# bittremieux/ANN-SoLo

Measured on AMD Instinct MI355X. Metric: query spectra/sec + recall@k vs brute-force, open-mod search on MassIVE-KB, higher is better.
Workload: dtype f32; 1 GPU; configs[2]: MassIVE-KB-scale synthetic library (2100000 spectra, one charge-2 partition), ivfpq m=32 nlist=4096 nprobe=128 k=1024, open +-500 Da, shifted dot, fragment tol 0.02 Da; library_size=2100000, batch_per_gpu=32768, reference_default_batch_size=16384, global_batch=32768, index=ivfpq, nlist=4096, nprobe=128, k=1024, parallelism=single

## Files before the change

ann_solo_amd/csrc/pq_scan_v3.hip:

```cpp
#include "common.hpp"
#include "hist_topk.hpp"
#include "ivf_kernels.hpp"
#include "pq_tile.hpp"

namespace asl {

constexpr int V3_CHUNK = 256;
constexpr int V3_DEPTH = 1;
constexpr int V3_NT = 0;
constexpr int V3_AHEAD = 8;
constexpr uint32_t V3_MM_DEAD = 0xfffffff0u;
constexpr int V3_PAD_SALU = 0;
constexpr int V3_PAD_VALU = 0;
#define V3_PAD4(op) op " %0, 0\n\t" op " %1, 1\n\t" op " %2, 2\n\t" op " %3, 3\n\t"
#define V3_PAD16(op) V3_PAD4(op) V3_PAD4(op) V3_PAD4(op) V3_PAD4(op)
template <int NS_, int NV_>
__device__ __forceinline__ void v3_pad() {
  static_assert(NS_ % 16 == 0 && NV_ % 16 == 0, "the padding comes in blocks of 16 instructions");
#pragma unroll
  for (int n = 0; n < NS_ / 16; ++n) {
    uint32_t a, b, c, d;
    asm volatile(V3_PAD16("s_mov_b32") : "=s"(a), "=s"(b), "=s"(c), "=s"(d));
  }
#pragma unroll
  for (int n = 0; n < NV_ / 16; ++n) {
    uint32_t a, b, c, d;
    asm volatile(V3_PAD16("v_mov_b32") : "=v"(a), "=v"(b), "=v"(c), "=v"(d));
  }
}
#undef V3_PAD16
#undef V3_PAD4
constexpr int V3_PAD_LDSRT = 0;
template <int N_>
__device__ __forceinline__ void v3_pad_ldsrt(const int *word) {
  if constexpr (N_ > 0) {
    typedef __attribute__((address_space(3))) int lds_int;
    uint32_t a = (uint32_t)(uintptr_t)(const lds_int *)word;
#pragma unroll
    for (int n = 0; n < N_; ++n) {
      const int r = __builtin_amdgcn_readfirstlane(
          __hip_atomic_load((const lds_int *)(uintptr_t)a, __ATOMIC_RELAXED, __HIP_MEMORY_SCOPE_WORKGROUP));
      asm volatile("" : "+v"(a) : "s"(r));
    }
  }
}
constexpr int V3_WAVES_PER_SIMD = 6;

template <int NT_>
__device__ __forceinline__ uint4 load_codes16(const uint8_t *p) {
  if (NT_) {
    const uint32_t *w = reinterpret_cast<const uint32_t *>(p);
    typedef uint32_t u32x4 __attribute__((ext_vector_type(4)));
    const u32x4 v = __builtin_nontemporal_load(reinterpret_cast<const u32x4 *>(w));
    return make_uint4(v.x, v.y, v.z, v.w);
  }
  return *reinterpret_cast<const uint4 *>(p);
}

struct TileEnt8 {
  uint32_t tile_nv;
  float coarse;
};

struct TileEnt12 {
  uint32_t tile_nv;
  float coarse;
  uint32_t first;
};
constexpr int V3_CHUNK_RANGED = 168;
static_assert(V3_CHUNK_RANGED * sizeof(TileEnt12) <= V3_CHUNK * sizeof(TileEnt8), "the ranged table fits the 2 KB");

template <int CAP, int T, int NW, int DEPTH, bool WIDE, bool RANGED = false, bool SEL = false, bool MM = false>
__global__ __launch_bounds__(64 * NW, (NW == 8 ? (CAP <= 2048 ? V3_WAVES_PER_SIMD : 4) : (CAP <= 2048 ? 3 : 1))) void pq_scan_v3_kernel(
    const float *__restrict__ xq, int d, const float *__restrict__ codebooks, int dsub,
    const float *__restrict__ coarse_D, const int32_t *__restrict__ coarse_I, int nprobe,
    const int32_t *__restrict__ list_offsets, const int32_t *__restrict__ tile_offsets,
    const uint8_t *__restrict__ codes_tiled, const int32_t *__restrict__ ids_tiled, int k,
    float *__restrict__ D, int64_t *__restrict__ I64, int32_t *__restrict__ I32, int set_mode,
    const uint2 *__restrict__ ent, const int32_t *__restrict__ ent_cnt, const int *__restrict__ gate,
    const ScanPostFilter pf, const ScanRanges rg, const unsigned long long *__restrict__ sel, const uint32_t mm_plane) {
  static_assert(!SEL || CAP <= 2048, "the selector is built into the 2048-key instantiations only");
  static_assert(!MM || (!RANGED && !SEL), "the sub-quantiser-major copy exists of the default layout only");
  if (gate && (int)blockIdx.x >= *gate) return;
  static_assert(DEPTH >= 1 && DEPTH <= 3, "rounds of prefetch");
  static_assert(T == 1, "one tile per wave at a time (two lost on registers: profiles/HISTORY.md)");
  constexpr int NT = 64 * NW, ROUND_VECS = NW * 64;
  using TopK = HistTopK<CAP, ROUND_VECS, NT>;
  using Ent = typename std::conditional<RANGED, TileEnt12, TileEnt8>::type;
  extern __shared__ __attribute__((aligned(16))) char smem[];
  float *s_lut = reinterpret_cast<float *>(smem + TopK::lds_bytes());
  Ent *table = reinterpret_cast<Ent *>(s_lut + PQT_KSUB * PQT_M);
  float *s_q = reinterpret_cast<float *>(smem);

  const int tid = threadIdx.x, lane = tid & 63, wave = tid >> 6, q = blockIdx.x;
  constexpr int PP = WIDE ? 2 : 1;
  int my_len[PP], my_tile0[PP], my_nt[PP], my_pre[PP];
  float my_coarse[PP];
#pragma unroll
  for (int pp = 0; pp < PP; ++pp) {
    my_len[pp] = 0, my_tile0[pp] = 0, my_nt[pp] = 0, my_coarse[pp] = 0.0f;
    const int p = tid + pp * NT;
    if (p < nprobe) {
      const int l = coarse_I[(size_t)q * nprobe + p];
      if (l >= 0) {
        if constexpr (RANGED) {
          const int2 r = rg.range[(size_t)q * nprobe + p];
          my_len[pp] = r.y > r.x ? r.y - (r.x & ~63) : 0;
          my_tile0[pp] = (int)((uint32_t)(tile_offsets[l] + (r.x >> 6)) | ((uint32_t)(r.x & 63) << 26));
        } else {
          my_len[pp] = list_offsets[l + 1] - list_offsets[l];
          my_tile0[pp] = tile_offsets[l];
        }
        my_nt[pp] = (my_len[pp] + 63) >> 6;
        my_coarse[pp] = coarse_D[(size_t)q * nprobe + p];
      }
    }
  }
  build_lut_cbt<NT>(xq + (size_t)q * d, d, codebooks, dsub, s_q, s_lut, reinterpret_cast<uint8_t *>(table),
                    tid, ent ? ent + (size_t)q * 64 : nullptr,
                    ent ? (xq ? ent_cnt[q] : max(ent_cnt[q], 0)) : -1);

  uint32_t live_u = 0;
  if constexpr (MM) {
    const uint8_t *s_nz = reinterpret_cast<const uint8_t *>(table);
    const int K = reinterpret_cast<const int *>(s_nz)[0];
    uint32_t mine = 0;
    for (int i = tid & 63; i < K; i += 64) mine |= 1u << (s_nz[8 + i] & 31);
#pragma unroll
    for (int o = 32; o > 0; o >>= 1) mine |= (uint32_t)__shfl_xor((int)mine, o);
    live_u = (uint32_t)__builtin_amdgcn_readfirstlane((int)mine);
    __syncthreads();
  }

  int total = 0;
  int *scan_part = reinterpret_cast<int *>(table);
#pragma unroll
  for (int pp = 0; pp < PP; ++pp) {
    int part_total;
    my_pre[pp] = total + block_excl_scan<NW>(my_nt[pp], scan_part, tid, part_total);
    total += part_total;
    __syncthreads();
  }
  total = __builtin_amdgcn_readfirstlane(total);

  TopK top;
  top.init(smem, k, ids_tiled, tid);
  top.out_keys = set_mode == 2 && I64 != nullptr;

  const char *lut_bytes = reinterpret_cast<const char *>(s_lut);
  const int wave_u = __builtin_amdgcn_readfirstlane(wave);
  const int rho = lane >> 4, j = lane & 15;
  const int ma = (rho & 1) ? j + 16 : j, mb = ma ^ 16;
  const uint32_t offA = (uint32_t)ma * 4u, offB = (uint32_t)mb * 4u;
  const bool liveA = (live_u >> ma) & 1u, liveB = (live_u >> mb) & 1u;
  const uint32_t chunkA = MM ? (liveA ? (uint32_t)ma * mm_plane + (uint32_t)(rho * 16) : V3_MM_DEAD) : (uint32_t)(rho * 512 + ma * 16);
  const uint32_t chunkB = liveB ? (uint32_t)mb * mm_plane + (uint32_t)(rho * 16) : V3_MM_DEAD;

  int *s_flag = top.ctl + TopK::C_USER;
  int *s_done = top.ctl + TopK::C_USER + 1;
  if (tid == 0) {
    *s_flag = 0;
    *s_done = 0;
  }
  auto flag_up = [&]() -> int { return __hip_atomic_load(s_flag, __ATOMIC_RELAXED, __HIP_MEMORY_SCOPE_WORKGROUP); };
  auto flag_set = [&](int v) { __hip_atomic_store(s_flag, v, __ATOMIC_RELAXED, __HIP_MEMORY_SCOPE_WORKGROUP); };
  float thr_u = -INFINITY;
  uint32_t thr_hi_u = 0;
  int flag_u = 0;

  constexpr int CHUNK = RANGED ? V3_CHUNK_RANGED : V3_CHUNK;
  for (int c0 = 0; c0 < total; c0 += CHUNK) {
#pragma unroll
    for (int pp = 0; pp < PP; ++pp) {
      asm volatile("" : "+v"(my_pre[pp]), "+v"(my_tile0[pp]), "+v"(my_len[pp]));
      const int lo = max(my_pre[pp], c0), hi = min(my_pre[pp] + ((my_len[pp] + 63) >> 6), c0 + CHUNK);
      for (int t = lo; t < hi; ++t) {
        const int local = t - my_pre[pp];
        Ent e;
        const uint32_t tile0 = RANGED ? (uint32_t)my_tile0[pp] & 0x3ffffffu : (uint32_t)my_tile0[pp];
        e.tile_nv = (tile0 + (uint32_t)local) | ((uint32_t)(min(64, my_len[pp] - local * 64) - 1) << 26);
        e.coarse = my_coarse[pp];
        if constexpr (RANGED) e.first = local == 0 ? (uint32_t)my_tile0[pp] >> 26 : 0u;
        table[t - c0] = e;
      }
    }
    __syncthreads();
    const int nent = min(CHUNK, total - c0);
    constexpr int NS = DEPTH + 1;
    uint4 A[NS], B[NS];
    if constexpr (MM) {
#pragma unroll
      for (int s = 0; s < NS; ++s) A[s] = B[s] = make_uint4(0u, 0u, 0u, 0u);
    }
    struct Tile {
      uint32_t tile_nv;
      float coarse;
      uint32_t first;
      unsigned long long sel;
    } e[NS];
    auto fetch = [&](uint32_t taddr, uint4 &a, uint4 &b, Tile &en, uint32_t num_records = 0) {
      typedef uint32_t u32x2 __attribute__((ext_vector_type(2)));
      const u32x2 t = *(const __attribute__((address_space(3))) u32x2 *)(uintptr_t)taddr;
      en.tile_nv = __builtin_amdgcn_readfirstlane(t.x);
      en.coarse = __builtin_bit_cast(float, __builtin_amdgcn_readfirstlane((int)t.y));
      if constexpr (RANGED)
        en.first = __builtin_amdgcn_readfirstlane(*(const __attribute__((address_space(3))) uint32_t *)(uintptr_t)(taddr + 8u));
      if constexpr (SEL) en.sel = sel[en.tile_nv & 0x3ffffffu];
      if constexpr (MM) {
        const uint32_t toff = (en.tile_nv & 0x3ffffffu) * 64u;
        const uint8_t *base = codes_tiled + (size_t)toff;
        const __amdgpu_buffer_rsrc_t rs =
            __builtin_amdgcn_make_buffer_rsrc(const_cast<uint8_t *>(base), 0, (int)num_records, 0x00020000);
        typedef uint32_t u32x4 __attribute__((ext_vector_type(4)));
        const u32x4 va = __builtin_amdgcn_raw_buffer_load_b128(rs, (int)chunkA, 0, V3_NT ? 2 : 0);
        const u32x4 vb = __builtin_amdgcn_raw_buffer_load_b128(rs, (int)chunkB, 0, V3_NT ? 2 : 0);
        a = make_uint4(va.x, va.y, va.z, va.w);
        b = make_uint4(vb.x, vb.y, vb.z, vb.w);
      } else {
        const uint8_t *base = codes_tiled + (size_t)(en.tile_nv & 0x3ffffffu) * 2048;
        uint32_t offa = chunkA;
        asm volatile("" : "+v"(offa));
        const uint32_t offb = offa ^ 256u;
        a = load_codes16<V3_NT>(base + offa);
        b = load_codes16<V3_NT>(base + offb);
      }
    };
    constexpr uint32_t ENT_STRIDE = NW * sizeof(Ent);
    const uint32_t mm_size = (uint32_t)PQT_M * mm_plane;
    float p_score = 0.0f;
    uint32_t p_tile_nv = 0, p_first = 0;
    unsigned long long p_sel = 0;
    bool pending = false;
    auto in_mask = [&]() -> unsigned long long {
      unsigned long long in = ~0ull >> (~(p_tile_nv >> 26) & 63u);
      if constexpr (RANGED) in &= ~0ull << (p_first & 63u);
      if constexpr (SEL) in &= p_sel;
      return in;
    };
    auto passers = [&]() -> unsigned long long { return __ballot(p_score >= thr_u) & in_mask(); };
    auto append = [&](unsigned long long m, bool hot = false) {
      if (!hot && thr_hi_u != 0) {
        float sc = p_score;
        asm volatile("; exact flushes" : "+v"(sc));
        m = __ballot(f2ord(sc) >= thr_hi_u) & in_mask();
      }
      pending = false;
      if (hot || m) {
        const int c = __builtin_amdgcn_readfirstlane(__popcll(m));
        const int base = top.reserve_add(c);
        pending = base + c > CAP;
        if (!pending) top.free_write(__builtin_amdgcn_inverse_ballot_w64(m), m, p_score, (p_tile_nv << 6) + (uint32_t)lane, base, false);
      }
    };
    const uint32_t table_lds = (uint32_t)(uintptr_t)(const __attribute__((address_space(3))) char *)reinterpret_cast<const char *>(table);
    int i = wave_u;
    if (i < nent) {
      uint32_t t0 = table_lds + (uint32_t)i * (uint32_t)sizeof(Ent);
      asm volatile("" : "+v"(t0));
#pragma unroll
      for (int s = 0; s < DEPTH; ++s)
        if (i + s * NW < nent) fetch(t0 + s * ENT_STRIDE, A[s], B[s], e[s], mm_size);
    }
    uint32_t taddr = 0;
    auto step = [&](int s) {
      const int f = (s + DEPTH) % NS;
      const int fl = flag_up();
      const bool real = i + DEPTH * NW < nent;
      if constexpr (MM) {
        taddr += real ? ENT_STRIDE : 0u;
        fetch(taddr, A[f], B[f], e[f], real ? mm_size : 0u);
      } else if (real) {
        taddr += ENT_STRIDE;
        fetch(taddr, A[f], B[f], e[f]);
      }
      flag_u = __builtin_amdgcn_readfirstlane(fl);
      p_score = e[s].coarse + tile_adc<V3_AHEAD>(lut_bytes, A[s], B[s], offA, offB);
      p_tile_nv = e[s].tile_nv;
      if constexpr (RANGED) p_first = e[s].first;
      if constexpr (SEL) p_sel = e[s].sel;
      i += NW;
    };
    auto hot = [&]() -> int {
      for (;;) {
#pragma unroll
        for (int s = 0; s < NS; ++s) {
          if (i >= nent) return -1;
          step(s);
          v3_pad<V3_PAD_SALU, V3_PAD_VALU>();
          v3_pad_ldsrt<V3_PAD_LDSRT>(s_done);
          const unsigned long long m = passers();
          if (__builtin_expect(((uint32_t)m | (uint32_t)(m >> 32) | (uint32_t)flag_u | thr_hi_u) != 0u, 0)) {
            if (((uint32_t)flag_u | thr_hi_u) != 0u) return s;
            append(m, true);
            if (pending) return s + NS;
          }
        }
      }
    };
    bool finished = false;
    for (;;) {
      taddr = table_lds + (uint32_t)(DEPTH == 1 ? min(i, CHUNK - 1) : min(i + (DEPTH - 1) * NW, nent - 1)) * (uint32_t)sizeof(Ent);
      asm volatile("" : "+v"(taddr));
      int ev = hot();
      asm volatile("" : "+s"(ev));
      bool meet = false;
#pragma unroll
      for (int s = 0; s < NS; ++s) {
        if (ev < 0 || s < ev % NS || meet) continue;
        if (s > ev % NS) {
          if (i >= nent) continue;
          step(s);
        }
        if (!(ev >= NS && s == ev % NS)) append(passers());
        if (pending || flag_u) {
          meet = true;
          if (s + 1 < NS) {
#pragma unroll
            for (int u = 0; u < DEPTH; ++u) {
              A[u] = A[(s + 1 + u) % NS];
              B[u] = B[(s + 1 + u) % NS];
              e[u] = e[(s + 1 + u) % NS];
            }
          }
        }
      }
      if (ev >= 0 && !meet) continue;
      if (!meet) {
        if (!finished) {
          if (lane == 0) atomicAdd(s_done, 1);
          finished = true;
        }
        for (;;) {
          flag_u = __builtin_amdgcn_readfirstlane(flag_up());
          if (flag_u ||
              __builtin_amdgcn_readfirstlane(__hip_atomic_load(s_done, __ATOMIC_RELAXED, __HIP_MEMORY_SCOPE_WORKGROUP)) >=
                  NW * (c0 / CHUNK + 1))
            break;
          __builtin_amdgcn_s_sleep(4);
        }
        if (!flag_u) break;
      }
      do {
        if (lane == 0) flag_set(1);
        __syncthreads();
        if (tid == 0) flag_set(0);
        asm volatile("" : "+v"(top.tid));
        top.free_sync(true);
        thr_u = __builtin_bit_cast(float, __builtin_amdgcn_readfirstlane(__builtin_bit_cast(int, top.thr_f)));
        thr_hi_u = (uint32_t)__builtin_amdgcn_readfirstlane((int)top.thr_hi);
        flag_u = 0;
        if (pending) append(passers());
      } while (pending);
    }
    __syncthreads();
  }
  top.free_done(true);
  if constexpr (RANGED) {
    if (set_mode) {
      const int n = top.finish_set(D ? D + (size_t)q * k : nullptr, I64 ? I64 + (size_t)q * k : nullptr,
                                   I32 ? I32 + (size_t)q * k : nullptr, reinterpret_cast<u64 *>(s_lut));
      if (rg.row_len && tid == 0) rg.row_len[q] = n;
    } else {
      top.finish(D ? D + (size_t)q * k : nullptr, I64 ? I64 + (size_t)q * k : nullptr,
                 I32 ? I32 + (size_t)q * k : nullptr);
    }
  } else if (set_mode && CAP * 9 <= PQT_KSUB * PQT_M * 4)
    top.finish_set(D ? D + (size_t)q * k : nullptr, I64 ? I64 + (size_t)q * k : nullptr,
                   I32 ? I32 + (size_t)q * k : nullptr, reinterpret_cast<u64 *>(s_lut), &pf, q);
  else if (set_mode && CAP * 8 <= PQT_KSUB * PQT_M * 4)
    top.finish_set(D ? D + (size_t)q * k : nullptr, I64 ? I64 + (size_t)q * k : nullptr,
                   I32 ? I32 + (size_t)q * k : nullptr, reinterpret_cast<u64 *>(s_lut));
  else
    top.finish(D ? D + (size_t)q * k : nullptr, I64 ? I64 + (size_t)q * k : nullptr,
               I32 ? I32 + (size_t)q * k : nullptr);
}

template <int CAP, int T, int NW, int DEPTH, bool WIDE, bool RANGED = false, bool SEL = false, bool MM = false>
static int launch_v3(const float *xq, int nq, int d, const float *codebooks, int dsub,
                     const float *coarse_D, const int32_t *coarse_I, int nprobe,
                     const int32_t *list_offsets, const int32_t *tile_offsets,
                     const uint8_t *codes_tiled, const int32_t *ids_tiled, int k, float *D,
                     int64_t *I64, int32_t *I32, int set_mode, const uint2 *ent,
                     const int32_t *ent_cnt, const int *gate, const ScanPostFilter &pf,
                     const ScanRanges &rg, const unsigned long long *sel = nullptr, uint32_t mm_plane = 0) {
  constexpr size_t TABLE = RANGED ? V3_CHUNK_RANGED * sizeof(TileEnt12) : V3_CHUNK * sizeof(TileEnt8);
  if ((size_t)d * 4 > (size_t)CAP * 8 || dsub > 64 || (size_t)d * 2 + 8 > TABLE || d != PQT_M * dsub)
    return fail(ASL_ERR_CAPACITY, "pq scan: d=%d too large for the LDS staging", d);
  const size_t lds = HistTopK<CAP, NW * T * 64, 64 * NW>::lds_bytes() + (size_t)PQT_KSUB * PQT_M * 4 +
                     (size_t)V3_CHUNK * sizeof(TileEnt8);
  if (lds > 160 * 1024) return fail(ASL_ERR_CAPACITY, "pq scan: k=%d does not fit LDS", k);
  if (lds > 64 * 1024)
    HIP_TRY(hipFuncSetAttribute((const void *)pq_scan_v3_kernel<CAP, T, NW, DEPTH, WIDE, RANGED, SEL, MM>,
                                hipFuncAttributeMaxDynamicSharedMemorySize, (int)lds));
  hipLaunchKernelGGL((pq_scan_v3_kernel<CAP, T, NW, DEPTH, WIDE, RANGED, SEL, MM>), dim3(nq), dim3(64 * NW), lds, stream(),
                     xq, d, codebooks, dsub, coarse_D, coarse_I, nprobe, list_offsets, tile_offsets,
                     codes_tiled, ids_tiled, k, D, I64, I32, set_mode, ent, ent_cnt, gate, pf, rg, sel, mm_plane);
  ASL_CHECK_LAUNCH();
  return ASL_OK;
}

bool pq_scan_tiled_supported(int m, int ksub, int k, int nprobe) {
  return m == PQT_M && ksub == PQT_KSUB && nprobe <= 1024 && k >= 1 && k <= TK_MAX_K;
}

int pq_scan_v3(const float *xq, int nq, int d, const float *codebooks, int dsub,
               const float *coarse_D, const int32_t *coarse_I, int nprobe,
               const int32_t *list_offsets, const int32_t *tile_offsets,
               const uint8_t *codes_tiled, const int32_t *ids_tiled, int k, float *D,
               int64_t *I64, int32_t *I32, int set_mode, const uint2 *ent, const int32_t *ent_cnt,
               const int *gate, const ScanPostFilter *post, const ScanRanges *ranges,
               const unsigned long long *sel, const uint8_t *codes_mm, uint32_t mm_plane) {
  if (nq <= 0) return ASL_OK;
  ScanPostFilter pf;
  if (post && post->idpay) {
    if (!(set_mode == 1 && I32 && k + 256 + 512 <= 2048))
      return fail(ASL_ERR_STATE, "pq scan: a post-filter needs set-mode int32 rows and k <= 1280");
    pf = *post;
  }
  const ScanRanges none;
#define V3_ARGS xq, nq, d, codebooks, dsub, coarse_D, coarse_I, nprobe, list_offsets, tile_offsets, \
                codes_tiled, ids_tiled, k, D, I64, I32, set_mode, ent, ent_cnt, gate, pf
  if (sel && (set_mode == 2 || k + 256 + 512 > 2048))
    return fail(ASL_ERR_STATE, "pq scan: a selector needs k <= 1280 and rows of ids");
  if (ranges && ranges->range) {
    if (pf.idpay || set_mode == 2 || k + 256 + 512 > 2048)
      return fail(ASL_ERR_STATE, "pq scan: the window scan needs k <= 1280, rows of ids and no post-filter");
    if (sel) {
      if (nprobe > 512) return launch_v3<2048, 1, 8, V3_DEPTH, true, true, true>(V3_ARGS, *ranges, sel);
      return launch_v3<2048, 1, 8, V3_DEPTH, false, true, true>(V3_ARGS, *ranges, sel);
    }
    if (nprobe > 512) return launch_v3<2048, 1, 8, V3_DEPTH, true, true>(V3_ARGS, *ranges);
    return launch_v3<2048, 1, 8, V3_DEPTH, false, true>(V3_ARGS, *ranges);
  }
  if (sel) {
    if (nprobe > 512) return launch_v3<2048, 1, 8, V3_DEPTH, true, false, true>(V3_ARGS, none, sel);
    return launch_v3<2048, 1, 8, V3_DEPTH, false, false, true>(V3_ARGS, none, sel);
  }
  if (codes_mm && !gate) {
#define V3_MM_ARGS xq, nq, d, codebooks, dsub, coarse_D, coarse_I, nprobe, list_offsets, tile_offsets, \
                   codes_mm, ids_tiled, k, D, I64, I32, set_mode, ent, ent_cnt, gate, pf, none, nullptr, mm_plane
    if (nprobe > 512) {
      if (k + 256 + 512 <= 2048) return launch_v3<2048, 1, 8, V3_DEPTH, true, false, false, true>(V3_MM_ARGS);
      return launch_v3<4096, 1, 8, V3_DEPTH, true, false, false, true>(V3_MM_ARGS);
    }
    if (k + 256 + 512 <= 2048) return launch_v3<2048, 1, 8, V3_DEPTH, false, false, false, true>(V3_MM_ARGS);
    return launch_v3<4096, 1, 8, V3_DEPTH, false, false, false, true>(V3_MM_ARGS);
#undef V3_MM_ARGS
  }
  if (nprobe > 512) {
    if (k + 256 + 512 <= 2048) return launch_v3<2048, 1, 8, V3_DEPTH, true>(V3_ARGS, none);
    return launch_v3<4096, 1, 8, V3_DEPTH, true>(V3_ARGS, none);
  }
  if (k + 256 + 512 <= 2048) return launch_v3<2048, 1, 8, V3_DEPTH, false>(V3_ARGS, none);
  return launch_v3<4096, 1, 8, V3_DEPTH, false>(V3_ARGS, none);
#undef V3_ARGS
}

__global__ void window_ranges_kernel(const double *__restrict__ q_pmz, int nq,
                                     const int32_t *__restrict__ coarse_I, int nprobe,
                                     const int32_t *__restrict__ list_offsets,
                                     const int32_t *__restrict__ tile_offsets,
                                     const float *__restrict__ wkey, int charge, double tol, int mode,
                                     int2 *__restrict__ ranges, unsigned long long *__restrict__ acc) {
  const int64_t i = block_linear() * blockDim.x + threadIdx.x;
  unsigned long long cnt = 0;
  if (i < (int64_t)nq * nprobe) {
    const int l = coarse_I[i];
    int2 r = make_int2(0, 0);
    if (l >= 0) {
      const float *key = wkey + (size_t)tile_offsets[l] * 64;
      const int n = list_offsets[l + 1] - list_offsets[l];
      r = window_run(key, n, query_window(q_pmz, i / nprobe, mode), charge, tol, mode);
      cnt = (unsigned long long)(r.y - r.x);
    }
    ranges[i] = r;
  }
  if (acc) {
    for (int off = 32; off > 0; off >>= 1) cnt += __shfl_xor(cnt, off);
    if ((threadIdx.x & 63) == 0 && cnt) atomicAdd(acc, cnt);
  }
}

int window_ranges(const double *q_pmz, int nq, const int32_t *coarse_I, int nprobe,
                  const int32_t *list_offsets, const int32_t *tile_offsets, const float *wkey, int charge,
                  double tol, int mode, int2 *ranges, unsigned long long *acc) {
  const int64_t n = (int64_t)nq * nprobe;
  if (n <= 0) return ASL_OK;
  hipLaunchKernelGGL(window_ranges_kernel, grid_2d(cdiv(n, 256)), dim3(256), 0, stream(), q_pmz, nq, coarse_I,
                     nprobe, list_offsets, tile_offsets, wkey, charge, tol, mode, ranges, acc);
  ASL_CHECK_LAUNCH();
  return ASL_OK;
}

__global__ void tile_codes_kernel(const uint8_t *__restrict__ codes, const int32_t *__restrict__ ids,
                                  const int32_t *__restrict__ dst_slot, int64_t n,
                                  uint8_t *__restrict__ codes_tiled,
                                  int32_t *__restrict__ ids_tiled) {
  const int64_t t = block_linear() * blockDim.x + threadIdx.x;
  if (t >= n * PQT_M) return;
  const int64_t i = t >> 5;
  const int m = (int)(t & 31);
  const int32_t slot = dst_slot[i];
  const int64_t tile = slot >> 6;
  const int v = slot & 63, rho = v >> 4, b = (v & 15) ^ (m & 15);
  codes_tiled[tile * 2048 + rho * 512 + m * 16 + b] = codes[t];
  if (m == 0) ids_tiled[tile * 64 + v] = ids[i];
}

int tile_codes(const uint8_t *codes, const int32_t *ids, const int32_t *dst_slot, int64_t n,
               int64_t ntiles, uint8_t *codes_tiled, int32_t *ids_tiled) {
  HIP_TRY(hipMemsetAsync(codes_tiled, 0, (size_t)ntiles * 2048, stream()));
  HIP_TRY(hipMemsetAsync(ids_tiled, 0xff, (size_t)ntiles * 64 * 4, stream()));
  if (n <= 0) return ASL_OK;
  hipLaunchKernelGGL(tile_codes_kernel, grid_2d(cdiv(n * PQT_M, 256)), dim3(256), 0,
                     stream(), codes, ids, dst_slot, n, codes_tiled, ids_tiled);
  ASL_CHECK_LAUNCH();
  return ASL_OK;
}

__global__ void mmajor_codes_kernel(const uint4 *__restrict__ codes_tiled, int64_t ntiles, uint32_t plane,
                                    uint8_t *__restrict__ codes_mm) {
  const int64_t t = block_linear() * blockDim.x + threadIdx.x;
  if (t >= ntiles * 128) return;
  const int64_t tile = t >> 7;
  const int rho = (int)(t >> 5) & 3, m = (int)(t & 31);
  *reinterpret_cast<uint4 *>(codes_mm + (size_t)m * plane + (size_t)tile * 64 + rho * 16) = codes_tiled[t];
}

int mmajor_codes(const uint8_t *codes_tiled, int64_t ntiles, uint32_t plane, uint8_t *codes_mm) {
  HIP_TRY(hipMemsetAsync(codes_mm, 0, (size_t)plane * PQT_M, stream()));
  if (ntiles <= 0) return ASL_OK;
  hipLaunchKernelGGL(mmajor_codes_kernel, grid_2d(cdiv(ntiles * 128, 256)), dim3(256), 0, stream(),
                     reinterpret_cast<const uint4 *>(codes_tiled), ntiles, plane, codes_mm);
  ASL_CHECK_LAUNCH();
  return ASL_OK;
}

__global__ __launch_bounds__(256) void tile_selector_kernel(const int32_t *__restrict__ slot_ids, int64_t ntiles,
                                                            const uint8_t *__restrict__ keep, int64_t n,
                                                            unsigned long long *__restrict__ words) {
  const int64_t tile = block_linear() * 4 + (threadIdx.x >> 6);
  const int lane = threadIdx.x & 63;
  if (tile >= ntiles) return;
  const int32_t id = slot_ids[tile * 64 + lane];
  const unsigned long long m = __ballot(id >= 0 && id < n && keep[id] != 0);
  if (lane == 0) words[tile] = m;
}

int tile_selector(const int32_t *slot_ids, int64_t ntiles, const uint8_t *keep, int64_t n,
                  unsigned long long *words) {
  if (ntiles <= 0) return ASL_OK;
  hipLaunchKernelGGL(tile_selector_kernel, grid_2d(cdiv(ntiles, 4)), dim3(256), 0, stream(), slot_ids, ntiles,
                     keep, n, words);
  ASL_CHECK_LAUNCH();
  return ASL_OK;
}

}
```

Baseline: 3.031 million query spectra/s.

## Hand out whole probe lists to waves via an LDS ticket in the MM scan

In the sub-quantiser-major scan path, the block-wide prefix scan and per-tile table expansion are replaced by a compact per-probe table. Each wave claims an entire inverted list through an LDS atomic ticket and walks its tiles sequentially. This removes the scan barriers and the per-tile table writes, and makes tile addresses consecutive within a wave. The cost is an atomic per list claim and possible load imbalance when list lengths vary, and the path is restricted to nprobe >= 32.

```diff
diff --git a/ann_solo_amd/csrc/pq_scan_v3.hip b/ann_solo_amd/csrc/pq_scan_v3.hip
--- a/ann_solo_amd/csrc/pq_scan_v3.hip
+++ b/ann_solo_amd/csrc/pq_scan_v3.hip
@@ -69,6 +69,15 @@
 };
 constexpr int V3_CHUNK_RANGED = 168;
 static_assert(V3_CHUNK_RANGED * sizeof(TileEnt12) <= V3_CHUNK * sizeof(TileEnt8), "the ranged table fits the 2 KB");
+
+struct ProbeEnt {
+  uint32_t tile0;
+  int32_t len;
+  float coarse;
+  uint32_t pad;
+};
+constexpr int V3_CHUNK_PROBES = 128;
+static_assert(V3_CHUNK_PROBES * sizeof(ProbeEnt) <= V3_CHUNK * sizeof(TileEnt8), "the probe table fits the 2 KB");
 
 template <int CAP, int T, int NW, int DEPTH, bool WIDE, bool RANGED = false, bool SEL = false, bool MM = false>
 __global__ __launch_bounds__(64 * NW, (NW == 8 ? (CAP <= 2048 ? V3_WAVES_PER_SIMD : 4) : (CAP <= 2048 ? 3 : 1))) void pq_scan_v3_kernel(
@@ -86,7 +95,7 @@
   static_assert(T == 1, "one tile per wave at a time (two lost on registers: profiles/HISTORY.md)");
   constexpr int NT = 64 * NW, ROUND_VECS = NW * 64;
   using TopK = HistTopK<CAP, ROUND_VECS, NT>;
-  using Ent = typename std::conditional<RANGED, TileEnt12, TileEnt8>::type;
+  using Ent = typename std::conditional<RANGED, TileEnt12, typename std::conditional<MM, ProbeEnt, TileEnt8>::type>::type;
   extern __shared__ __attribute__((aligned(16))) char smem[];
   float *s_lut = reinterpret_cast<float *>(smem + TopK::lds_bytes());
   Ent *table = reinterpret_cast<Ent *>(s_lut + PQT_KSUB * PQT_M);
@@ -111,7 +120,7 @@
           my_len[pp] = list_offsets[l + 1] - list_offsets[l];
           my_tile0[pp] = tile_offsets[l];
         }
-        my_nt[pp] = (my_len[pp] + 63) >> 6;
+        if constexpr (!MM) my_nt[pp] = (my_len[pp] + 63) >> 6;
         my_coarse[pp] = coarse_D[(size_t)q * nprobe + p];
       }
     }
@@ -132,16 +141,18 @@
     __syncthreads();
   }
 
-  int total = 0;
-  int *scan_part = reinterpret_cast<int *>(table);
-#pragma unroll
-  for (int pp = 0; pp < PP; ++pp) {
-    int part_total;
-    my_pre[pp] = total + block_excl_scan<NW>(my_nt[pp], scan_part, tid, part_total);
-    total += part_total;
-    __syncthreads();
-  }
-  total = __builtin_amdgcn_readfirstlane(total);
+  int total = MM ? nprobe : 0;
+  if constexpr (!MM) {
+    int *scan_part = reinterpret_cast<int *>(table);
+#pragma unroll
+    for (int pp = 0; pp < PP; ++pp) {
+      int part_total;
+      my_pre[pp] = total + block_excl_scan<NW>(my_nt[pp], scan_part, tid, part_total);
+      total += part_total;
+      __syncthreads();
+    }
+    total = __builtin_amdgcn_readfirstlane(total);
+  }
 
   TopK top;
   top.init(smem, k, ids_tiled, tid);
@@ -158,6 +169,7 @@
 
   int *s_flag = top.ctl + TopK::C_USER;
   int *s_done = top.ctl + TopK::C_USER + 1;
+  int *s_ticket = top.ctl + TopK::C_USER + 2;
   if (tid == 0) {
     *s_flag = 0;
     *s_done = 0;
@@ -168,20 +180,32 @@
   uint32_t thr_hi_u = 0;
   int flag_u = 0;
 
-  constexpr int CHUNK = RANGED ? V3_CHUNK_RANGED : V3_CHUNK;
+  constexpr int CHUNK = RANGED ? V3_CHUNK_RANGED : MM ? V3_CHUNK_PROBES : V3_CHUNK;
   for (int c0 = 0; c0 < total; c0 += CHUNK) {
-#pragma unroll
-    for (int pp = 0; pp < PP; ++pp) {
-      asm volatile("" : "+v"(my_pre[pp]), "+v"(my_tile0[pp]), "+v"(my_len[pp]));
-      const int lo = max(my_pre[pp], c0), hi = min(my_pre[pp] + ((my_len[pp] + 63) >> 6), c0 + CHUNK);
-      for (int t = lo; t < hi; ++t) {
-        const int local = t - my_pre[pp];
-        Ent e;
-        const uint32_t tile0 = RANGED ? (uint32_t)my_tile0[pp] & 0x3ffffffu : (uint32_t)my_tile0[pp];
-        e.tile_nv = (tile0 + (uint32_t)local) | ((uint32_t)(min(64, my_len[pp] - local * 64) - 1) << 26);
-        e.coarse = my_coarse[pp];
-        if constexpr (RANGED) e.first = local == 0 ? (uint32_t)my_tile0[pp] >> 26 : 0u;
-        table[t - c0] = e;
+    if constexpr (MM) {
+#pragma unroll
+      for (int pp = 0; pp < PP; ++pp) {
+        const uint32_t local = (uint32_t)(tid + pp * NT - c0);
+        if (local < (uint32_t)CHUNK)
+          *reinterpret_cast<uint4 *>(&table[local]) =
+              make_uint4((uint32_t)my_tile0[pp], (uint32_t)my_len[pp], __float_as_uint(my_coarse[pp]), 0u);
+      }
+      if (tid == 0) __hip_atomic_store(s_ticket, 0, __ATOMIC_RELAXED, __HIP_MEMORY_SCOPE_WORKGROUP);
+    }
+    if constexpr (!MM) {
+#pragma unroll
+      for (int pp = 0; pp < PP; ++pp) {
+        asm volatile("" : "+v"(my_pre[pp]), "+v"(my_tile0[pp]), "+v"(my_len[pp]));
+        const int lo = max(my_pre[pp], c0), hi = min(my_pre[pp] + ((my_len[pp] + 63) >> 6), c0 + CHUNK);
+        for (int t = lo; t < hi; ++t) {
+          const int local = t - my_pre[pp];
+          Ent e;
+          const uint32_t tile0 = RANGED ? (uint32_t)my_tile0[pp] & 0x3ffffffu : (uint32_t)my_tile0[pp];
+          e.tile_nv = (tile0 + (uint32_t)local) | ((uint32_t)(min(64, my_len[pp] - local * 64) - 1) << 26);
+          e.coarse = my_coarse[pp];
+          if constexpr (RANGED) e.first = local == 0 ? (uint32_t)my_tile0[pp] >> 26 : 0u;
+          table[t - c0] = e;
+        }
       }
     }
     __syncthreads();
@@ -198,14 +222,7 @@
       uint32_t first;
       unsigned long long sel;
     } e[NS];
-    auto fetch = [&](uint32_t taddr, uint4 &a, uint4 &b, Tile &en, uint32_t num_records = 0) {
-      typedef uint32_t u32x2 __attribute__((ext_vector_type(2)));
-      const u32x2 t = *(const __attribute__((address_space(3))) u32x2 *)(uintptr_t)taddr;
-      en.tile_nv = __builtin_amdgcn_readfirstlane(t.x);
-      en.coarse = __builtin_bit_cast(float, __builtin_amdgcn_readfirstlane((int)t.y));
-      if constexpr (RANGED)
-        en.first = __builtin_amdgcn_readfirstlane(*(const __attribute__((address_space(3))) uint32_t *)(uintptr_t)(taddr + 8u));
-      if constexpr (SEL) en.sel = sel[en.tile_nv & 0x3ffffffu];
+    auto load_tile = [&](uint4 &a, uint4 &b, const Tile &en, uint32_t num_records) {
       if constexpr (MM) {
         const uint32_t toff = (en.tile_nv & 0x3ffffffu) * 64u;
         const uint8_t *base = codes_tiled + (size_t)toff;
@@ -225,8 +242,63 @@
         b = load_codes16<V3_NT>(base + offb);
       }
     };
+    auto fetch = [&](uint32_t taddr, uint4 &a, uint4 &b, Tile &en) {
+      typedef uint32_t u32x2 __attribute__((ext_vector_type(2)));
+      const u32x2 t = *(const __attribute__((address_space(3))) u32x2 *)(uintptr_t)taddr;
+      en.tile_nv = __builtin_amdgcn_readfirstlane(t.x);
+      en.coarse = __builtin_bit_cast(float, __builtin_amdgcn_readfirstlane((int)t.y));
+      if constexpr (RANGED)
+        en.first = __builtin_amdgcn_readfirstlane(*(const __attribute__((address_space(3))) uint32_t *)(uintptr_t)(taddr + 8u));
+      if constexpr (SEL) en.sel = sel[en.tile_nv & 0x3ffffffu];
+      load_tile(a, b, en, 0u);
+    };
     constexpr uint32_t ENT_STRIDE = NW * sizeof(Ent);
     const uint32_t mm_size = (uint32_t)PQT_M * mm_plane;
+    uint32_t cur_tile = 0, cur_last = 0, nx_tile = 0, nx_last = 0;
+    int cur_left = 0, nx_left = 0;
+    float cur_coarse = 0.0f, nx_coarse = 0.0f;
+    int inflight = 0;
+    auto take_list = [&]() {
+      typedef __attribute__((address_space(3))) int lds_int;
+      typedef uint32_t u32x4 __attribute__((ext_vector_type(4)));
+      nx_left = 0;
+      nx_tile = 0;
+      for (;;) {
+        uint32_t ta = (uint32_t)(uintptr_t)(lds_int *)s_ticket;
+        asm volatile("" : "+v"(ta));
+        int t = (int)ta;
+        if (lane == 0)
+          t = __hip_atomic_fetch_add((lds_int *)(uintptr_t)ta, 1, __ATOMIC_RELAXED, __HIP_MEMORY_SCOPE_WORKGROUP);
+        t = __builtin_amdgcn_readfirstlane(t);
+        if (t >= nent) break;
+        const u32x4 v = *(const __attribute__((address_space(3))) u32x4 *)(uintptr_t)(
+            (uint32_t)(uintptr_t)(const __attribute__((address_space(3))) char *)reinterpret_cast<const char *>(table) +
+            (uint32_t)t * (uint32_t)sizeof(ProbeEnt));
+        const int len = __builtin_amdgcn_readfirstlane((int)v.y);
+        if (len > 0) {
+          nx_tile = (uint32_t)__builtin_amdgcn_readfirstlane((int)v.x);
+          nx_coarse = __builtin_bit_cast(float, __builtin_amdgcn_readfirstlane((int)v.z));
+          nx_left = (len + 63) >> 6;
+          nx_last = (uint32_t)(len - 1) & 63u;
+          break;
+        }
+      }
+    };
+    auto next_list = [&]() {
+      cur_tile = nx_tile, cur_left = nx_left, cur_coarse = nx_coarse, cur_last = nx_last;
+      if (cur_left != 0) take_list();
+    };
+    auto fetch_mm = [&](uint4 &a, uint4 &b, Tile &en) {
+      const bool real = cur_left != 0;
+      en.tile_nv = cur_tile | ((cur_left == 1 ? cur_last : 63u) << 26);
+      en.coarse = cur_coarse;
+      load_tile(a, b, en, real ? mm_size : 0u);
+      if (real) {
+        ++inflight;
+        ++cur_tile;
+        if (--cur_left == 0) next_list();
+      }
+    };
     float p_score = 0.0f;
     uint32_t p_tile_nv = 0, p_first = 0;
     unsigned long long p_sel = 0;
@@ -254,22 +326,29 @@
     };
     const uint32_t table_lds = (uint32_t)(uintptr_t)(const __attribute__((address_space(3))) char *)reinterpret_cast<const char *>(table);
     int i = wave_u;
-    if (i < nent) {
+    if constexpr (MM) {
+      take_list();
+      next_list();
+#pragma unroll
+      for (int s = 0; s < DEPTH; ++s)
+        if (cur_left != 0) fetch_mm(A[s], B[s], e[s]);
+    } else if (i < nent) {
       uint32_t t0 = table_lds + (uint32_t)i * (uint32_t)sizeof(Ent);
       asm volatile("" : "+v"(t0));
 #pragma unroll
       for (int s = 0; s < DEPTH; ++s)
-        if (i + s * NW < nent) fetch(t0 + s * ENT_STRIDE, A[s], B[s], e[s], mm_size);
-    }
+        if (i + s * NW < nent) fetch(t0 + s * ENT_STRIDE, A[s], B[s], e[s]);
+    }
+    auto more = [&]() -> bool { return MM ? inflight != 0 : i < nent; };
     uint32_t taddr = 0;
     auto step = [&](int s) {
       const int f = (s + DEPTH) % NS;
       const int fl = flag_up();
-      const bool real = i + DEPTH * NW < nent;
       if constexpr (MM) {
-        taddr += real ? ENT_STRIDE : 0u;
-        fetch(taddr, A[f], B[f], e[f], real ? mm_size : 0u);
-      } else if (real) {
+        fetch_mm(A[f], B[f], e[f]);
+        --inflight;
+        asm volatile("" : "+s"(inflight));
+      } else if (i + DEPTH * NW < nent) {
         taddr += ENT_STRIDE;
         fetch(taddr, A[f], B[f], e[f]);
       }
@@ -284,7 +363,7 @@
       for (;;) {
 #pragma unroll
         for (int s = 0; s < NS; ++s) {
-          if (i >= nent) return -1;
+          if (!more()) return -1;
           step(s);
           v3_pad<V3_PAD_SALU, V3_PAD_VALU>();
           v3_pad_ldsrt<V3_PAD_LDSRT>(s_done);
@@ -299,8 +378,10 @@
     };
     bool finished = false;
     for (;;) {
-      taddr = table_lds + (uint32_t)(DEPTH == 1 ? min(i, CHUNK - 1) : min(i + (DEPTH - 1) * NW, nent - 1)) * (uint32_t)sizeof(Ent);
-      asm volatile("" : "+v"(taddr));
+      if constexpr (!MM) {
+        taddr = table_lds + (uint32_t)(DEPTH == 1 ? min(i, CHUNK - 1) : min(i + (DEPTH - 1) * NW, nent - 1)) * (uint32_t)sizeof(Ent);
+        asm volatile("" : "+v"(taddr));
+      }
       int ev = hot();
       asm volatile("" : "+s"(ev));
       bool meet = false;
@@ -308,7 +389,7 @@
       for (int s = 0; s < NS; ++s) {
         if (ev < 0 || s < ev % NS || meet) continue;
         if (s > ev % NS) {
-          if (i >= nent) continue;
+          if (!more()) continue;
           step(s);
         }
         if (!(ev >= NS && s == ev % NS)) append(passers());
@@ -436,7 +517,7 @@
     if (nprobe > 512) return launch_v3<2048, 1, 8, V3_DEPTH, true, false, true>(V3_ARGS, none, sel);
     return launch_v3<2048, 1, 8, V3_DEPTH, false, false, true>(V3_ARGS, none, sel);
   }
-  if (codes_mm && !gate) {
+  if (codes_mm && !gate && nprobe >= 32) {
 #define V3_MM_ARGS xq, nq, d, codebooks, dsub, coarse_D, coarse_I, nprobe, list_offsets, tile_offsets, \
                    codes_mm, ids_tiled, k, D, I64, I32, set_mode, ent, ent_cnt, gate, pf, none, nullptr, mm_plane
     if (nprobe > 512) {
```

Result: faster. 3.082 million query spectra/s (median of 6 runs) (+1.7%).
